# rishabhgoel0213/ZeroClone

Hardware: AMD Instinct MI355X
Metric: MCTS node-expansions/sec (whole node), Connect4 800 sims/move at 1/2/4/8 MI355X (higher is better)
Workload: dtype f64

## Files before the change

zeroclone_amd/csrc/c4_device.h:

```cpp
#pragma once
#include <math.h>

#include "c4_order_table.h"
#include "zc_internal.h"

namespace zc {
namespace {

__constant__ uint32_t d_order[128] = {ZC_C4_ORDER_LIST};

constexpr uint32_t kRingMask = kRingWords - 1;
constexpr uint64_t kBottom = 0x0000040810204081ull;
constexpr uint64_t kFull = kBottom * 0x3Full;
constexpr uint64_t kTop = kBottom << 5;
constexpr int kTabBytes = 128 * 4 + 128 * 8;

__device__ __forceinline__ uint32_t untried_init(uint32_t n) { return ((1u << n) - 1u) | (n << 28); }
__device__ __forceinline__ uint32_t untried_count(uint32_t u) { return (uint32_t)__popc(u & 0x7Fu); }

__device__ __forceinline__ void load_tables(uint32_t *s_order) {
    for (int i = (int)threadIdx.x; i < 128; i += blockDim.x) s_order[i] = d_order[i];
    uint8_t *const s_sel = (uint8_t *)(s_order + 128);
    for (int i = (int)threadIdx.x; i < 1024; i += blockDim.x) {
        const uint32_t m = (uint32_t)i >> 3, r = (uint32_t)i & 7u;
        uint32_t c = 0, pos = 7;
        for (uint32_t b = 0; b < 7; ++b)
            if ((m >> b) & 1u) {
                if (c == r) {
                    pos = b;
                    break;
                }
                ++c;
            }
        s_sel[i] = (uint8_t)pos;
    }
}
__device__ __forceinline__ const uint8_t *sel_table(const uint32_t *s_order) { return (const uint8_t *)(s_order + 128); }
constexpr int kWin = 64;
constexpr int kPathSpill = 2 * (64 - kMaxDepth) + 24;

__device__ __forceinline__ uint32_t uni(uint32_t x) { return (uint32_t)__builtin_amdgcn_readfirstlane((int)x); }
__device__ __forceinline__ int uni(int x) { return __builtin_amdgcn_readfirstlane(x); }
__device__ __forceinline__ uint64_t uni64(uint64_t x) {
    return ((uint64_t)uni((uint32_t)(x >> 32)) << 32) | (uint64_t)uni((uint32_t)x);
}
__device__ __forceinline__ uint32_t lane_id() { return __lane_id(); }
__device__ __forceinline__ uint32_t mask_sel(uint64_t m, uint32_t a, uint32_t b) {
    uint32_t r;
    __asm__("v_cndmask_b32 %0, %1, %2, %3" : "=v"(r) : "v"(a), "v"(b), "s"(m));
    return r;
}
__device__ __forceinline__ uint32_t mask_sel0(uint64_t m, uint32_t b) {
// ... 152 lines not shown

__device__ __forceinline__ uint32_t rng_view(const Rng &r) {
    const uint32_t lane = lane_id();
    const uint32_t src = lane < r.off ? r.wn : r.wt;
    return (uint32_t)__builtin_amdgcn_ds_bpermute((int)((lane + r.off) << 2), (int)src);
}

__device__ __forceinline__ void rng_close(const Rng &r, uint64_t use0, uint64_t *rngpos) {
    rngpos[0] = use0 + (uint64_t)(int64_t)r.use();
    rngpos[1] = use0 + (uint64_t)(int64_t)r.grel;
}

constexpr int kLRingWords = 1024;
constexpr uint32_t kLRingMask = kLRingWords - 1;
constexpr int kLRingBytes = kLRingWords * 4;

struct LRng {
    uint32_t *lds;
    uint32_t base;
    int32_t wrel;
    uint32_t off;
    int32_t hrel;
    uint32_t wa, wb;
    uint64_t ph;
    __device__ __forceinline__ uint32_t cur() const { return mask_sel(ph, wa, wb); }
    uint32_t wx;
    uint32_t ia, ib, im;
    __device__ __forceinline__ int32_t use() const { return wrel + (int32_t)off; }
    __device__ __forceinline__ uint32_t slot(int32_t rel) const { return (base + (uint32_t)rel) & kLRingMask; }
};

__device__ __forceinline__ uint32_t mt_twist(uint32_t a, uint32_t b, uint32_t m) {
    const uint32_t y = (a & 0x80000000u) | (b & 0x7fffffffu);
    return m ^ (y >> 1) ^ ((b & 1u) ? 0x9908b0dfu : 0u);
}

__device__ __forceinline__ void lrng_prefetch(LRng &r) {
    const int32_t p = r.wrel + 192 + (int32_t)lane_id();
    r.ia = r.lds[r.slot(p - 624)];
    r.ib = r.lds[r.slot(p - 623)];
    r.im = r.lds[r.slot(p - 227)];
}

__device__ __forceinline__ void lrng_generate_abs(uint32_t *lds, uint64_t g, uint64_t end) {
    const uint32_t lane = lane_id();
    for (; g < end; g += 64) {
        const uint32_t p = (uint32_t)g + lane;
        const uint32_t a = lds[(p - 624) & kLRingMask], b = lds[(p - 623) & kLRingMask],
                       m = lds[(p - 227) & kLRingMask];
        if (g + lane < end) lds[p & kLRingMask] = mt_twist(a, b, m);
        wave_mem_order();
    }
}

__device__ __forceinline__ void lrng_open(LRng &r, uint32_t *lds, const uint32_t *ring, uint64_t use0, uint64_t gen0) {
    const uint32_t lane = lane_id();
    r.lds = lds;
    r.base = (uint32_t)use0;
    r.off = (uint32_t)use0 & (uint32_t)(kWin - 1);
    r.wrel = -(int32_t)r.off;
    const uint64_t w0 = use0 - r.off, target = w0 + 192;
    const uint64_t g = gen0 <= w0 + 960 ? gen0 : (target < 624 ? 624 : target);
    for (uint32_t i = lane; i < (uint32_t)kLRingWords; i += 64) {
        const uint32_t p = (uint32_t)g - (uint32_t)kLRingWords + i;
        lds[p & kLRingMask] = ring[p & kRingMask];
    }
    wave_mem_order();
    lrng_generate_abs(lds, g, target);
    r.hrel = (int32_t)(g - use0);
    r.wa = temper(lds[r.slot(r.wrel + (int32_t)lane)]);
    r.wb = temper(lds[r.slot(r.wrel + kWin + (int32_t)lane)]);
    r.ph = 0;
    r.wx = lds[r.slot(r.wrel + 2 * kWin + (int32_t)lane)];
    lrng_prefetch(r);
}

__device__ __forceinline__ uint32_t rng_view(const LRng &r) {
    const uint32_t lane = lane_id();
    const uint32_t src = mask_sel(__ballot(lane < r.off) ^ r.ph, r.wa, r.wb);
    return (uint32_t)__builtin_amdgcn_ds_bpermute((int)((lane + r.off) << 2), (int)src);
}

__device__ __forceinline__ void rng_advance(LRng &r) {
    r.wrel += kWin;
    r.off -= (uint32_t)kWin;
    const uint32_t t = temper(r.wx);
    const uint32_t na = mask_sel(r.ph, t, r.wa), nb = mask_sel(r.ph, r.wb, t);
    r.wa = na;
    r.wb = nb;
    r.ph = ~r.ph;
    const int32_t p = r.wrel + 128 + (int32_t)lane_id();
    uint32_t x = mt_twist(r.ia, r.ib, r.im);
    if (r.wrel + 128 < r.hrel) {
        const uint32_t old = r.lds[r.slot(p)];
        x = p < r.hrel ? old : x;
    }
    r.lds[r.slot(p)] = x;
    r.wx = x;
    lrng_prefetch(r);
}

__device__ __forceinline__ void lrng_skip(LRng &r, uint32_t w) {
    r.off += w;
    while (r.off >= (uint32_t)kWin) rng_advance(r);
}

__device__ __forceinline__ void lrng_close(const LRng &r, uint32_t *ring, uint64_t use0, uint64_t *rngpos) {
    const uint32_t lane = lane_id();
    const uint64_t U = use0 + (uint64_t)(int64_t)r.use();
    uint64_t G = use0 + (uint64_t)(int64_t)max(r.wrel + 192, r.hrel);
    const uint64_t blk = U ? (U - 1) / 624 : 0;
    const uint64_t bend = (blk + 1) * 624;
    wave_mem_order();
    if (G < bend) {
        lrng_generate_abs(r.lds, G, bend);
        G = bend;
    }
    const uint64_t wu = U & ~(uint64_t)(kWin - 1);
    uint64_t start = wu < blk * 624 ? wu : blk * 624;
    start = start < G - 624 ? start : G - 624;
    for (uint64_t q = start + lane; q < G; q += 64) ring[(uint32_t)q & kRingMask] = r.lds[(uint32_t)q & kLRingMask];
    if (lane == 0) {
        rngpos[0] = U;
        rngpos[1] = G;
    }
}

template <class R>
__device__ __forceinline__ uint32_t rng_below(R &r, uint32_t n) {
    const uint32_t sh = (uint32_t)__clz(n);
    const uint32_t lane = lane_id();
    for (;;) {
        if (r.off >= (uint32_t)kWin) rng_advance(r);
        const uint32_t v = r.cur() >> sh;
        const uint64_t bal = __ballot((v | ((lane - r.off) & 0x80000000u)) < n);
        if (bal) {
// ... 254 lines not shown
            if (lane == (uint32_t)depth) pathv = (uint32_t)child | ((uint32_t)s << 16);
            node = child;
            ow = (uint32_t)__builtin_amdgcn_readlane((int)c_low, i);
            cmask = __builtin_amdgcn_readlane((int)c_lmask, i);
            u = untried_init((ow >> 24) & 15u);
            ul = kIdentList;
            ch = 0xFFFF;
            stamp.mark(2);
            continue;
        }
        const int m = min((int)cnt, nb - j);
        uint32_t rr = 0;
        {
            int done = 0;
            for (;;) {
                if (rng.off >= (uint32_t)kWin) rng_advance(rng);
                const uint32_t w = rng_view(rng);
                const int rem = m - done;
                uint64_t A[7];
#pragma unroll
                for (int i = 0; i < 7; ++i) {
                    const uint32_t n = (uint32_t)max((int)cnt - done - i, 1);
                    A[i] = __ballot((w >> __clz(n)) < n);
                }
                uint64_t gt = ~0ull, F = 0;
#pragma unroll
                for (int i = 0; i < 7; ++i) {
                    const uint64_t acc = (i < rem ? A[i] : 0ull) & gt;
                    const uint64_t lb = acc & (0ull - acc);
                    F |= lb;
                    gt = 0ull - (lb << 1);
                }
                const int nd = __popcll(F);
                const int f = 63 - __clzll(F | 1ull);
                const uint32_t di = (uint32_t)done + mbcnt64(F);
                const uint32_t rl = w >> __clz(max((int)cnt - (int)di, 1));
                const uint32_t got = (uint32_t)__builtin_amdgcn_ds_permute((int)(mask_sel(F, 63u, di) << 2), (int)rl);
                rr = mask_sel(((1ull << nd) - 1ull) << done, rr, got);
                done += nd;
                if (done < m) {
                    rng.off += (uint32_t)kWin;
                    continue;
                }
                rng.off += (uint32_t)f + 1u;
                break;
            }
        }
        uint32_t pl = rr;
        uint32_t rpick[6];
#pragma unroll
        for (int i = 0; i < 6; ++i) rpick[i] = (uint32_t)__builtin_amdgcn_readlane((int)rr, i);
#pragma unroll
        for (int i = 5; i >= 0; --i) {
            const uint64_t later = ((1ull << m) - 1ull) & ~((2ull << i) - 1ull);
            pl = add_in_mask(pl, __ballot(pl >= rpick[i]) & later);
        }
        const uint32_t mi_l = (ul >> (3 * (pl & 7u))) & 7u;
        uint32_t slotbit = (int)lane < m ? 1u << mi_l : 0u;
        slotbit |= (uint32_t)dpp<0xB1>((int)slotbit);
// ... 68 lines not shown
```

zeroclone_amd/csrc/c4_ext.hip:

```cpp
#include <hip/hip_fp16.h>

#include "c4_device.h"

namespace zc {
namespace {

__device__ __forceinline__ uint32_t mbcnt_lo(uint64_t m) {
    return __builtin_amdgcn_mbcnt_hi((uint32_t)(m >> 32), __builtin_amdgcn_mbcnt_lo((uint32_t)m, 0u));
}

__device__ __forceinline__ Tree ext_tree(const ExtParams &p, int g) {
    return Tree{p.a.nodes + (size_t)g * p.M * kRecBytes};
}

__global__ __launch_bounds__(kBlock) void c4_ext_begin_kernel(ExtParams p) {
    const uint32_t lane = lane_id();
    const int gl = blockIdx.x;
    if (gl >= p.n_games) return;
    const int g = p.first_game + gl;
    const zc_c4_state root = p.roots[gl];
    const uint64_t rp0 = uni64(root.stones[0]), rp1 = uni64(root.stones[1]);
    const int rturn = uni(root.turn);
    int status = 0;
    if (!valid_state(rp0, rp1, rturn)) status = ZC_STATUS_BAD_STATE;
// ... 332 lines not shown
}

void launch_c4_hp_walk(const ExtParams &p, hipStream_t s) {
    hipLaunchKernelGGL(c4_hp_walk_kernel, dim3(1), dim3(kBlock), 0, s, p);
}

void launch_c4_hp_expand(const ExtParams &p, hipStream_t s) {
    hipLaunchKernelGGL(c4_hp_expand_kernel, dim3(1), dim3(kBlock), 0, s, p);
}

void launch_c4_ext_begin(const ExtParams &p, hipStream_t s) {
    hipLaunchKernelGGL(c4_ext_begin_kernel, dim3(p.n_games), dim3(kBlock), 0, s, p);
}

void launch_c4_ext_select(const ExtParams &p, hipStream_t s) {
    hipLaunchKernelGGL(c4_ext_select_kernel, dim3(p.n_games), dim3(kBlock), c4_search_lds_bytes(p.bs), s, p);
}

void launch_c4_ext_backup(const ExtParams &p, hipStream_t s) {
    const size_t lds = (sizeof(double) + sizeof(int32_t)) * (size_t)p.bs;
    hipLaunchKernelGGL(c4_ext_backup_kernel, dim3(p.n_games), dim3(kBlock), lds, s, p);
}

void launch_c4_ext_end(const ExtParams &p, hipStream_t s) {
    hipLaunchKernelGGL(c4_ext_end_kernel, dim3(p.n_games), dim3(kBlock), 0, s, p);
}

}
```

zeroclone_amd/csrc/c4_search.hip:

```cpp
#include "c4_device.h"
#include "counter_rng.h"

namespace zc {
namespace {


__device__ __forceinline__ uint64_t readlane64(uint64_t x, int l) {
    return ((uint64_t)(uint32_t)__builtin_amdgcn_readlane((int)(x >> 32), l) << 32) |
           (uint64_t)(uint32_t)__builtin_amdgcn_readlane((int)x, l);
}

__device__ __forceinline__ uint32_t mbcnt(uint64_t m) {
    return __builtin_amdgcn_mbcnt_hi((uint32_t)(m >> 32), __builtin_amdgcn_mbcnt_lo((uint32_t)m, 0u));
}

__device__ __forceinline__ uint32_t scan_add32(uint32_t x) {
    x += (uint32_t)__builtin_amdgcn_update_dpp(0, (int)x, 0x111, 0xF, 0xF, false);
    x += (uint32_t)__builtin_amdgcn_update_dpp(0, (int)x, 0x112, 0xF, 0xF, false);
    x += (uint32_t)__builtin_amdgcn_update_dpp(0, (int)x, 0x114, 0xF, 0xF, false);
    x += (uint32_t)__builtin_amdgcn_update_dpp(0, (int)x, 0x118, 0xF, 0xF, false);
    x += (uint32_t)__builtin_amdgcn_update_dpp(0, (int)x, 0x142, 0xA, 0xF, false);
    x += (uint32_t)__builtin_amdgcn_update_dpp(0, (int)x, 0x143, 0xC, 0xF, false);
    return x;
}
// ... 44 lines not shown
    do {                                                            \
        if (ZC_RSTAMP && sub) {                                     \
            __builtin_amdgcn_sched_barrier(0);                      \
            const uint64_t now_ = __builtin_amdgcn_s_memtime();     \
            __builtin_amdgcn_sched_barrier(0);                      \
            if (ZC_RSTAMP == (k)) *sub += now_ - t_;                \
            t_ = now_;                                              \
        }                                                           \
    } while (0)
template <class R>
__device__ void c4_rollouts(Leaf *L, int nb, R &rng, const uint32_t *s_order, Counters &cn,
                            uint64_t *sub = nullptr) {
    uint64_t t_ = ZC_RSTAMP && sub ? __builtin_amdgcn_s_memtime() : 0;
    const uint32_t lane = lane_id();
    const uint32_t lrow = lane >> 4;
    const uint64_t second_rows = __ballot((lrow & 1u) != 0);
    const uint32_t d1 = lrow < 2 ? 1u : 6u, d2 = lrow < 2 ? 7u : 8u;
    const uint32_t pairbits = lane < 49u ? (1u << (lane / 7u)) | (1u << (lane % 7u)) : 0u;
    __builtin_amdgcn_s_waitcnt(0x0F70);
    for (int g = 0; g < nb; g += 64) {
      uint32_t lm_v = 0, ow_v = 0, hp_v = 0;
      int room_v = 0;
      int val_v = 0, q_v = 0;
      {
        const int jj = g + (int)lane;
        if (jj < nb) {
            lm_v = L[jj].meta;
            ow_v = L[jj].ow;
            const uint64_t x0 = L[jj].p0, x1 = L[jj].p1;
            const uint64_t op_v = (lm_v >> 24) & 1u ? x0 : x1;
            room_v = has_four(op_v) ? -2 : 41 - __popcll(x0 | x1);
            const uint64_t oc = x0 | x1;
            for (int c = 0; c < 7; ++c) hp_v |= (uint32_t)__popcll((oc >> (7 * c)) & 0x3Full) << (4 * c);
#ifndef ZC_DIAG_WASTE
            cn.blocks += room_v >= 0 ? 1 : 0;
#endif
        }
      }
      const int jend = min(nb, g + 64);
      for (int j = g; j < jend; ++j) {
        RMARK(6);
        const int jl = j - g;
        const uint32_t lm = (uint32_t)__builtin_amdgcn_readlane((int)lm_v, jl);
        uint4 pw;
        __builtin_memcpy(&pw, &L[j], sizeof pw);
        uint64_t x0 = ((uint64_t)pw.y << 32) | pw.x, x1 = ((uint64_t)pw.w << 32) | pw.z;
        uint64_t S1 = (lm >> 24) & 1u ? ~second_rows : second_rows;
        uint32_t hp = (uint32_t)__builtin_amdgcn_readlane((int)hp_v, jl);
        const uint32_t low0 = (uint32_t)__builtin_amdgcn_readlane((int)ow_v, jl);
        const int room0 = __builtin_amdgcn_readlane(room_v, jl);
        int val = (room0 + 1) >> 1;
        int q = 0;
        RMARK(1);
        if (room0 >= 0) {
            int room = room0;
            int mask = (int)(lm >> 25);
            uint32_t ow = low0;
            uint32_t n = (ow >> 24) & 15u;
            uint32_t sh = (uint32_t)__builtin_clz(n);
            uint32_t owp = s_order[(uint32_t)mask & ~pairbits];
            uint32_t ew, l0, lf, endlane, endply, col, sc;
            uint64_t F, mine;
            auto block = [&]() __attribute__((always_inline)) {
                RMARK(6);
                uint32_t wv, v;
                uint64_t A;
                if (rng.off >= (uint32_t)kWin) rng_advance(rng);
                wv = rng_view(rng);
                v = wv >> sh;
                A = __ballot(v < n);
                if (__builtin_expect(A == 0ull, 0)) {
                    do {
                        rng.off += (uint32_t)kWin;
                        rng_advance(rng);
                        wv = rng_view(rng);
                        v = wv >> sh;
                        A = __ballot(v < n);
                    } while (A == 0ull);
                }
                RMARK(2);
                const uint32_t cap_r = min((uint32_t)room, 30u);
                uint32_t qk = mbcnt(A);
                col = (ow >> (3 * v)) & 7u;
                uint32_t one = mask_sel0(A, 1u << (4 * col));
                sc = scan_add32(one);
                uint32_t row = ((sc - one + hp) >> (4 * col)) & 15u;
                uint32_t nacc = (uint32_t)__popcll(A);
                F = __ballot(row == 5u);
                uint64_t E0 = A & (F | __ballot(qk >= min(cap_r, nacc - 1u)));
                l0 = (uint32_t)__builtin_ctzll(E0);
                const uint64_t G = A & F & __ballot(qk < cap_r);
                lf = ff1(G);
#ifdef ZC_DIAG_WASTE
                const uint32_t l0f = l0;
#endif
#if !(ZC_RV & 1)
                RMARK(3);
                if (lf == l0) {
                    const uint32_t cf = (uint32_t)__builtin_amdgcn_readlane((int)col, (int)lf);
                    const uint32_t ow2 = (uint32_t)__builtin_amdgcn_readlane((int)owp, (int)(8u * cf));
                    const uint32_t n2 = (ow2 >> 24) & 15u;
                    const uint32_t v2 = wv >> __clz(n2);
                    const uint64_t high = ~1ull << lf;
                    A = (A & ~high) | (__ballot(v2 < n2) & high);
                    qk = mbcnt(A);
                    col = mask_sel(high, col, (ow2 >> (3 * v2)) & 7u);
                    one = mask_sel0(A, 1u << (4 * col));
                    sc = scan_add32(one);
                    row = ((sc - one + hp) >> (4 * col)) & 15u;
                    nacc = (uint32_t)__popcll(A);
                    F = __ballot(row == 5u) & high;
                    E0 = A & (F | __ballot(qk >= min(cap_r, nacc - 1u)));
                    l0 = (uint32_t)__builtin_ctzll(E0);
                }
                RMARK(4);
                const uint32_t c = ((qk & 1u) << 4) | ((qk >> 1) & 15u) | (qk & 32u);
                const uint32_t b = __umul24(col, 7u) + row;
                const uint32_t pl = (uint32_t)__builtin_amdgcn_ds_permute((int)(mask_sel(A, 63u, c) << 2), (int)b);
                const uint32_t pb = __builtin_amdgcn_permlane32_swap(pl, pl, false, false)[0];
                const uint64_t bit = 1ull << (pb & 63u);
                uint32_t blo = (uint32_t)bit, bhi = (uint32_t)(bit >> 32);
// ... 21 lines not shown
                    x0 = in_vgpr(x0);
                    x1 = in_vgpr(x1);
                    const uint64_t bd = (((uint64_t)mask_sel(S1, (uint32_t)(x0 >> 32), (uint32_t)(x1 >> 32)) << 32) |
                                         mask_sel(S1, (uint32_t)x0, (uint32_t)x1)) | mine_;
                    const uint64_t m1 = bd & (bd >> d1), m2 = bd & (bd >> d2);
                    const uint64_t f4 = (m1 & (m1 >> (2 * d1))) | (m2 & (m2 >> (2 * d2)));
                    const uint64_t W = __ballot(f4 != 0ull);
                    const uint32_t W32 = (uint32_t)W | (uint32_t)(W >> 32);
                    return A_ & __ballot(((W32 >> (c & 31u)) & 1u) != 0u);
                };
                uint64_t Ew1 = 0, mine1 = 0;
                RMARK(3);
                if (lf == l0) {
                    const uint32_t cf = (uint32_t)__builtin_amdgcn_readlane((int)col, (int)lf);
                    const uint32_t ow2 = (uint32_t)__builtin_amdgcn_readlane((int)owp, (int)(8u * cf));
                    const uint32_t n2 = (ow2 >> 24) & 15u;
                    const uint32_t v2 = wv >> __clz(n2);
                    const uint64_t high = ~1ull << lf;
                    if (ZC_RV & 1) Ew1 = win_test(A, qk, col, row, mine1) & ~high;
                    A = (A & ~high) | (__ballot(v2 < n2) & high);
                    qk = mbcnt(A);
                    col = mask_sel(high, col, (ow2 >> (3 * v2)) & 7u);
                    one = mask_sel0(A, 1u << (4 * col));
                    sc = scan_add32(one);
                    row = ((sc - one + hp) >> (4 * col)) & 15u;
                    nacc = (uint32_t)__popcll(A);
                    F = __ballot(row == 5u) & high;
                    E0 = A & (F | __ballot(qk >= min(cap_r, nacc - 1u)));
                    l0 = (uint32_t)__builtin_ctzll(E0);
                }
                RMARK(4);
                uint64_t Ew;
                if ((ZC_RV & 1) && Ew1 != 0ull) {
                    Ew = Ew1;
                    mine = mine1;
                } else {
                    Ew = win_test(A, qk, col, row, mine);
                }
                if (ZC_RV & 1) Ew = uni64(Ew);
#endif
                ew = ff1(Ew);
                endlane = min(ew, l0);
                endply = (uint32_t)__builtin_amdgcn_readlane((int)qk, (int)endlane);
                rng.off += endlane + 1u;
#ifdef ZC_DIAG_WASTE
                cn.add(cn.blocks, lf == l0f && endlane < lf ? 1 : 0);
                cn.add(cn.plies, lf == l0f ? 1 : 0);
#endif
                room -= (int)endply + 1;
                RMARK(5);
                return neg_if_le(ew, l0, room);
            };
            auto go_on = [&]() __attribute__((always_inline)) {
#ifndef ZC_DIAG_WASTE
                cn.add(cn.blocks, 1);
#endif
                {
                    const uint64_t s2 = readlane64(mine, (int)((endply + 31u) >> 1));
                    const uint64_t a2 = readlane64(mine, (int)(endply >> 1));
// ... 1 lines not shown
                    const bool p1_first = S1 & 1ull;
                    x0 |= p1_first ? b2 : a2;
                    x1 |= p1_first ? a2 : b2;
                    S1 = endply & 1u ? S1 : ~S1;
                }
                hp += (uint32_t)__builtin_amdgcn_readlane((int)sc, (int)endlane);
                const bool fa = endlane >= lf;
                const bool fe = (F >> endlane) & 1u;
                {
                    const uint32_t ca = (uint32_t)__builtin_amdgcn_readlane((int)col, (int)(fa ? lf : endlane));
                    const uint32_t ce = fe ? (uint32_t)__builtin_amdgcn_readlane((int)col, (int)endlane) : ca;
                    const bool ff = fa | fe;
                    mask = ff ? mask & ~((1 << ca) | (1 << ce)) : mask;
                    const uint32_t ownew = (uint32_t)__builtin_amdgcn_readlane((int)owp, (int)((7u * ca + ce) & 63u));
                    ow = ff ? ownew : ow;
                    owp = s_order[(uint32_t)mask & ~pairbits];
                }
                n = (ow >> 24) & 15u;
                sh = (uint32_t)__builtin_clz(n);
            };
            if (block() >= 0) {
                do go_on();
                while (block() >= 0);
            }
            q = room0 - room;
            val = ew <= l0 ? ((q & 1) ? 1 : -1) : 0;
        }
        val_v = zc_writelane(val, jl, val_v);
        q_v = zc_writelane(q, jl, q_v);
      }
      if (g + (int)lane < jend) L[g + (int)lane].val = val_v;
#ifndef ZC_DIAG_WASTE
      cn.plies += q_v;
#endif
// ... 167 lines not shown
        return;
    }

    constexpr uint32_t kIdentList = 0x1AC688u;
    uint64_t b0 = we.b0, b1 = we.b1;
    int turn = we.turn, depth = we.depth;
    uint32_t ow = we.ow, cm = (uint32_t)legal_mask(b0 | b1), n = cnt0, ul = 0;
    {
        uint32_t k = 0;
        for (uint32_t bb = 0; bb < 7; ++bb)
            if ((we.u >> bb) & 1u) ul |= bb << (3 * k++);
    }
    int d = 0, i = 0, T = -1;
    uint64_t Sm = 0;
    uint32_t raw = 0;
    if (rng.off >= (uint32_t)kWin) rng_advance(rng);
    uint32_t w = rng_view(rng);
    uint32_t t3 = w >> 29;
    uint64_t gt = ~0ull, Fv = 0;
    int dv0 = 0;
    for (;;) {
        const int m = min((int)n, nb - d);
        if (lane == 0)
            chain[i] = ChainNode{b0, b1, ow,
                                 n | ((uint32_t)m << 4) | ((uint32_t)d << 8) | ((uint32_t)depth << 16) |
                                     ((uint32_t)turn << 24) | (cm << 25),
                                 ul, 0u};
        if (m == 0) {
            T = i;
            break;
        }
        Sm |= 1ull << d;
        int k = 0;
// ... 7 lines not shown
#pragma unroll
            for (int s = 0; s < 7; ++s) {
                const uint64_t acc = A[s] & gt;
                gt = (~1ull) << (ff1(acc) & 63u);
                F |= acc & ~gt;
            }
            Fv |= F;
            const int nd = __popcll(F);
            k += nd;
            d += nd;
            if (k < m) {
                const uint32_t di = (uint32_t)dv0 + mbcnt64(Fv);
                const uint32_t got =
                    (uint32_t)__builtin_amdgcn_ds_permute((int)(mask_sel(Fv, 63u, di) << 2), (int)w);
                raw = mask_sel(lanes_in(dv0, d), raw, got);
                rng.off += (uint32_t)kWin;
                rng_advance(rng);
                w = rng_view(rng);
                t3 = w >> 29;
                gt = ~0ull;
                Fv = 0;
                dv0 = d;
                continue;
            }
            gt = (~1ull) << (63 - __clzll(Fv));
            break;
        }
        if (d >= nb) break;
        const int col = (int)((ow >> (3 * (ul & 7u))) & 7u);
        const uint64_t bit = drop_bit(b0 | b1, col);
        if (turn) b1 |= bit; else b0 |= bit;
        turn ^= 1;
        ++depth;
        if (bit & kTop) {
            cm &= ~(1u << col);
            ow = uni(s_order[cm]);
        }
        n = (ow >> 24) & 15u;
        ul = kIdentList;
        ++i;
    }
    {
        const uint32_t di = (uint32_t)dv0 + mbcnt64(Fv);
        const uint32_t got = (uint32_t)__builtin_amdgcn_ds_permute((int)(mask_sel(Fv, 63u, di) << 2), (int)w);
        raw = mask_sel(lanes_in(dv0, d), raw, got);
        rng.off += (uint32_t)(63 - __clzll(Fv | 1ull)) + 1u;
    }
    const int D = d;
    wave_mem_order();
    stamp.mark(2);

    const bool act = (int)lane < D;
    const uint32_t seg = act ? mbcnt64(Sm) + (uint32_t)((Sm >> lane) & 1ull) - 1u : 0u;
    const ChainNode e = chain[seg];
    const uint32_t s_i = (e.info >> 8) & 0xFFu;
    const uint32_t dd = lane - s_i;
    const uint32_t r = raw >> __clz(act ? (e.info & 15u) - dd : 1u);
    uint32_t rp[6];
#pragma unroll
    for (int s = 0; s < 6; ++s) rp[s] = (uint32_t)__builtin_amdgcn_ds_bpermute((int)((s_i + (uint32_t)s) << 2), (int)r);
    uint32_t pl = r;
#pragma unroll
    for (int s = 5; s >= 0; --s) pl += (dd > (uint32_t)s && pl >= rp[s]) ? 1u : 0u;
    const uint32_t mi = (e.ul >> (3 * (pl & 7u))) & 7u;
    const uint64_t Z = __ballot(act && pl == 0);
    const uint64_t zl = Z & ((1ull << s_i) - 1ull);
    const int parent = seg == 0 ? we.node : f0 + 63 - __clzll(zl | 1ull);
    {
        const uint32_t col = (e.ow >> (3 * mi)) & 7u;
        const uint64_t bit = drop_bit(e.p0 | e.p1, (int)col);
        const uint32_t tn = (e.info >> 24) & 1u, ldepth = ((e.info >> 16) & 0xFFu) + 1u;
        const bool filled = (bit & kTop) != 0;
// ... 38 lines not shown
            const int q = base + (int)lane;
            const uint32_t dep = q < D ? fresh[q].link >> 24 : 0u;
#pragma unroll
            for (int bit = 0; bit < 6; ++bit) dsum += __popcll(__ballot((dep >> bit) & 1u)) << bit;
        }
        cn.add(cn.expansions, D);
        cn.add(cn.depth_sum, dsum);
    }
    stamp.mark(3);
}

__device__ __forceinline__ uint32_t draw_class_bfe(uint32_t cnt) {
    return (6u << 16) | (((0xE480u >> (2u * cnt)) & 3u) << 3);
}

__device__ __forceinline__ uint32_t draw_table(uint32_t w) {
    const uint32_t lane = lane_id();
    const uint32_t t3 = lane < 62u ? (w >> 29) : 7u;
    uint32_t nx = 0;
#pragma unroll
    for (uint32_t c = 0; c < 4; ++c) {
        const uint64_t s = __ballot(t3 < 4u + c) >> lane;
        const uint32_t f = s ? lane + 1u + (uint32_t)__builtin_ctzll(s) : 63u;
        nx |= f << (8u * c);
    }
    return nx;
}

__device__ __forceinline__ void write_lane(int &v, uint32_t x, int i) {
    __asm__("v_writelane_b32 %0, %1, m0" : "+v"(v) : "s"(x), "{m0}"(i));
}

__device__ __forceinline__ uint32_t draw_step(uint32_t nx, uint32_t q, uint32_t op) {
// ... 87 lines not shown
        ++i;
    }
    const int D = d;

    const bool act = (int)lane < D;
    const uint32_t seg = act ? mbcnt64(Sm) + (uint32_t)((Sm >> lane) & 1ull) - 1u : 0u;
    const int sa = (int)(seg << 2);
    const uint32_t e_cd = (uint32_t)__builtin_amdgcn_ds_bpermute(sa, v_cd);
    const uint32_t s_i = (e_cd >> 8) & 0xFFu;
    const uint32_t dd = lane - s_i;
    const uint32_t cnt = act ? (e_cd >> 16) - dd : 1u;
    const uint32_t clsv = draw_class_bfe(act ? cnt : 1u);

    uint32_t raw = 0;
    {
        if (rng.off >= (uint32_t)kWin) rng_advance(rng);
        uint32_t w = rng_view(rng);
        uint32_t nx = draw_table(w);
        int V = 0;
        uint64_t F = draw_chase_fixed<32>(nx, clsv);
        for (;;) {
            const uint64_t Fv = F & 0x7FFFFFFFFFFFFFFEull;
            const uint64_t G = Fv >> 1;
            const int nv = __popcll(G), need = D - V, take = min(nv, need);
            const uint32_t rank = mbcnt64(G);
            const bool send = ((G >> lane) & 1ull) && (int)rank < take;
            const uint32_t got = (uint32_t)__builtin_amdgcn_ds_permute(
                (int)((send ? (uint32_t)V + rank : 63u) << 2), (int)w);
            raw = mask_sel(lanes_in(V, V + take), raw, got);
            V += take;
            if (nv >= need) {
                const uint64_t lastw = __ballot(((G >> lane) & 1ull) && (int)rank == take - 1);
                rng.off += (uint32_t)__builtin_ctzll(lastw) + 1u;
                break;
            }
            uint32_t q;
            if (F >> 63) {
                rng.off += 62u;
                if (rng.off >= (uint32_t)kWin) rng_advance(rng);
                w = rng_view(rng);
                nx = draw_table(w);
                q = 0;
            } else {
                q = nv ? 64u - (uint32_t)__clzll(G) : 0u;
                rng.off += q;
                if (rng.off >= (uint32_t)kWin) rng_advance(rng);
                w = rng_view(rng);
                nx = draw_table(w);
                q = 0;
            }
            F = 0;
            for (int k = V; k < D; ++k) {
                q = draw_step(nx, q, (uint32_t)__builtin_amdgcn_readlane((int)clsv, k));
                F |= 1ull << q;
                if (q == 63u) break;
            }
        }
    }
    wave_mem_order();
    stamp.mark(2);

    const uint32_t e_ow = (uint32_t)__builtin_amdgcn_ds_bpermute(sa, v_ow);
    const uint64_t e_p0 = ((uint64_t)(uint32_t)__builtin_amdgcn_ds_bpermute(sa, v_b0h) << 32) |
                          (uint32_t)__builtin_amdgcn_ds_bpermute(sa, v_b0l);
    const uint64_t e_p1 = ((uint64_t)(uint32_t)__builtin_amdgcn_ds_bpermute(sa, v_b1h) << 32) |
                          (uint32_t)__builtin_amdgcn_ds_bpermute(sa, v_b1l);
    const uint32_t r = raw >> __clz(cnt);
    uint32_t rp[6];
#pragma unroll
    for (int s = 0; s < 6; ++s) rp[s] = (uint32_t)__builtin_amdgcn_ds_bpermute((int)((s_i + (uint32_t)s) << 2), (int)r);
    uint32_t pl = r;
#pragma unroll
    for (int s = 5; s >= 0; --s) pl += (dd > (uint32_t)s && pl >= rp[s]) ? 1u : 0u;
    const uint32_t mi = seg == 0 ? (uint32_t)sel_table(s_order)[8u * (we.u & 0x7Fu) + (pl & 7u)] : pl;
    const uint64_t Z = __ballot(act && pl == 0);
    const uint64_t zl = Z & ((1ull << s_i) - 1ull);
    const int parent = seg == 0 ? we.node : f0 + 63 - __clzll(zl | 1ull);
    {
        const uint32_t col = (e_ow >> (3 * mi)) & 7u;
        const uint64_t bit = drop_bit(e_p0 | e_p1, (int)col);
        const uint32_t tn = (uint32_t)we.turn ^ (seg & 1u), ldepth = (uint32_t)we.depth + seg + 1u;
        const bool filled = (bit & kTop) != 0;
// ... 42 lines not shown
    nnodes = f0 + D;
    wave_mem_order();
    {
        const uint32_t dep = act ? (uint32_t)we.depth + seg + 1u : 0u;
        int dsum = 0;
#pragma unroll
        for (int bit = 0; bit < 6; ++bit) dsum += __popcll(__ballot((dep >> bit) & 1u)) << bit;
        cn.add(cn.expansions, D);
        cn.add(cn.depth_sum, dsum);
    }
    stamp.mark(3);
}

constexpr int kSearchWaves = 4;
__host__ __device__ constexpr size_t c4_search_wave_lds(int bs) {
    return ((size_t)kLRingBytes + (sizeof(Leaf) + sizeof(Fresh) + sizeof(uint16_t) * kMaxDepth) * (size_t)bs +
            kPathSpill + 15) & ~(size_t)15;
}

struct SearchLds {
    uint32_t *s_order;
    uint32_t *ring;
    Fresh *fresh;
    Leaf *leaves;
    uint16_t *paths;
};

__device__ __forceinline__ SearchLds search_lds(uint8_t *s_dyn, int bs) {
    const uint32_t wave = threadIdx.x >> 6;
    uint8_t *const s_wave = s_dyn + kTabBytes + (size_t)wave * c4_search_wave_lds(bs);
    SearchLds L;
    L.s_order = (uint32_t *)s_dyn;
    L.ring = (uint32_t *)s_wave;
    L.fresh = (Fresh *)(s_wave + kLRingBytes);
    L.leaves = (Leaf *)(s_wave + kLRingBytes + sizeof(Fresh) * (size_t)bs);
    L.paths = (uint16_t *)(s_wave + kLRingBytes + (sizeof(Fresh) + sizeof(Leaf)) * (size_t)bs);
    return L;
}

template <bool STAMP, bool PHILOX, int WALK = 0>
__device__ __forceinline__ void search_move(const SearchParams &p, const SearchLds &L, int gl, int g, const Tree &t,
                                            LRng &rng, uint32_t tag, Counters &cn, int &status, int &done_io,
                                            int &nnodes_io, const int32_t *stop = nullptr, int32_t budget = 0,
                                            int *lagp = nullptr, const int32_t *progress = nullptr, int mv = 0) {
    int lag = lagp ? *lagp : 0;
    const uint32_t lane = lane_id();
    const uint32_t *const s_order = L.s_order;
    Fresh *const fresh = L.fresh;
    Leaf *const leaves = L.leaves;
    ConstDouble *logtab = (ConstDouble *)p.a.logtab;
    if (done_io == 0) {
// ... 11 lines not shown

        FlushSel fs;
        {
            const zc_c4_state root = p.roots[gl];
#ifndef ZC_NO_PLAN
#define ZC_NO_PLAN 0
#endif
#ifndef ZC_PLAN2
#define ZC_PLAN2 1
#endif
            if (!ZC_NO_PLAN && ZC_PLAN2 && p.bs < 64)
                select_flush_plan2<STAMP>(t, fresh, leaves, s_order, logtab, rng, cn, stamp, nnodes, status,
                                          uni64(root.stones[0]), uni64(root.stones[1]), uni(root.turn), done, nb,
                                          p.c, fs);
            else if (!ZC_NO_PLAN && p.bs < 64)
                select_flush_plan<STAMP>(t, fresh, leaves, (ChainNode *)L.paths, s_order, logtab, rng, cn, stamp,
                                         nnodes, status, uni64(root.stones[0]), uni64(root.stones[1]),
                                         uni(root.turn), done, nb, p.c, fs);
            else
                select_flush<false, STAMP>(t, fresh, leaves, nullptr, s_order, logtab, rng, cn, stamp, nnodes,
                                           status, uni64(root.stones[0]), uni64(root.stones[1]), uni(root.turn),
                                           done, nb, p.c, fs);
        }
        const int f0 = fs.f0, d0 = fs.d0;

        const size_t wlog = (size_t)g * p.sims + done;
        const size_t wfl = (size_t)g * ((p.sims + p.bs - 1) / p.bs) + done / p.bs;
        if (WALK == 2) {
            for (int jj = (int)lane; jj < nb; jj += kBlock) leaves[jj].val = p.walk_vals[wlog + jj];
            lrng_skip(rng, uni(p.walk_words[wfl]));
        } else if (PHILOX) {
// ... 540 lines not shown
```

Baseline: 3.436 billion.

## Precompute 3-bit tempered draws in LDS and refill MT ring in 4-word steps

Replaces the register-windowed Mersenne Twister reader with an LDS byte array of pre-tempered 3-bit draws (top bits of temper), so consumers read one byte per lane instead of tempering and bpermuting full words. The ring is refilled in batched steps of 224 words with 4 words per lane, and a new draw-order table is built at load time so move selection compares 3-bit draws against thresholds directly. It also changes the per-wave LDS layout and sizing. The cost is extra LDS per wave and more work in each refill step, which may limit occupancy; the ext_select launch now computes its LDS size separately from the shared helper.

```diff
diff --git a/zeroclone_amd/csrc/c4_device.h b/zeroclone_amd/csrc/c4_device.h
--- a/zeroclone_amd/csrc/c4_device.h
+++ b/zeroclone_amd/csrc/c4_device.h
@@ -13,13 +13,20 @@
 constexpr uint64_t kBottom = 0x0000040810204081ull;
 constexpr uint64_t kFull = kBottom * 0x3Full;
 constexpr uint64_t kTop = kBottom << 5;
-constexpr int kTabBytes = 128 * 4 + 128 * 8;
+constexpr int kTabBytes = 128 * 4 + 128 * 8 + 128 * 4;
 
 __device__ __forceinline__ uint32_t untried_init(uint32_t n) { return ((1u << n) - 1u) | (n << 28); }
 __device__ __forceinline__ uint32_t untried_count(uint32_t u) { return (uint32_t)__popc(u & 0x7Fu); }
 
 __device__ __forceinline__ void load_tables(uint32_t *s_order) {
-    for (int i = (int)threadIdx.x; i < 128; i += blockDim.x) s_order[i] = d_order[i];
+    for (int i = (int)threadIdx.x; i < 128; i += blockDim.x) {
+        const uint32_t o = d_order[i], n = (o >> 24) & 15u;
+        s_order[i] = o;
+        const uint32_t sh = n ? (uint32_t)__builtin_clz(n) - 29u : 0u;
+        uint32_t e = (n << sh) << 24;
+        for (uint32_t t = 0; t < (n << sh); ++t) e |= ((o >> (3u * (t >> sh))) & 7u) << (3u * t);
+        s_order[128 + 256 + i] = e;
+    }
     uint8_t *const s_sel = (uint8_t *)(s_order + 128);
     for (int i = (int)threadIdx.x; i < 1024; i += blockDim.x) {
         const uint32_t m = (uint32_t)i >> 3, r = (uint32_t)i & 7u;
@@ -36,6 +43,7 @@
     }
 }
 __device__ __forceinline__ const uint8_t *sel_table(const uint32_t *s_order) { return (const uint8_t *)(s_order + 128); }
+__device__ __forceinline__ const uint32_t *draw_order_table(const uint32_t *s_order) { return s_order + 128 + 256; }
 constexpr int kWin = 64;
 constexpr int kPathSpill = 2 * (64 - kMaxDepth) + 24;
 
@@ -218,35 +226,78 @@
 constexpr int kLRingWords = 1024;
 constexpr uint32_t kLRingMask = kLRingWords - 1;
 constexpr int kLRingBytes = kLRingWords * 4;
+constexpr int kLDrawBytes = kLRingWords + kWin;
+constexpr int kLStepLanes = 56;
+constexpr int kLStep = 4 * kLStepLanes;
+static_assert(kLStep <= 227 && kLStep % 4 == 0, "a refill step's inputs must all be older than its outputs");
+static_assert(kLRingWords - 624 - (kWin - 1 + kLStep) >= 0, "the block of word U-1 must stay in the ring");
+
+__host__ __device__ constexpr uint32_t mt_draw3(uint32_t x) {
+    const uint32_t y = x ^ (x >> 11);
+    const uint32_t z = y ^ ((y << 7) & 0x80004000u);
+    return (z ^ (z << 15)) >> 29;
+}
+__host__ __device__ constexpr uint32_t mt_temper_ref(uint32_t y) {
+    y ^= y >> 11;
+    y ^= (y << 7) & 0x9d2c5680u;
+    y ^= (y << 15) & 0xefc60000u;
+    y ^= y >> 18;
+    return y;
+}
+__host__ __device__ constexpr bool mt_draw3_matches_temper() {
+    if (mt_draw3(0u) != mt_temper_ref(0u) >> 29) return false;
+    for (int b = 0; b < 32; ++b)
+        if (mt_draw3(1u << b) != mt_temper_ref(1u << b) >> 29) return false;
+    return true;
+}
+static_assert(mt_draw3_matches_temper(), "mt_draw3 is not temper(x) >> 29");
 
 struct LRng {
     uint32_t *lds;
-    uint32_t base;
-    int32_t wrel;
-    uint32_t off;
-    int32_t hrel;
-    uint32_t wa, wb;
-    uint64_t ph;
-    __device__ __forceinline__ uint32_t cur() const { return mask_sel(ph, wa, wb); }
-    uint32_t wx;
-    uint32_t ia, ib, im;
-    __device__ __forceinline__ int32_t use() const { return wrel + (int32_t)off; }
-    __device__ __forceinline__ uint32_t slot(int32_t rel) const { return (base + (uint32_t)rel) & kLRingMask; }
+    const uint8_t *dl;
+    int32_t urel;
+    int32_t lim;
+    int32_t uoff;
+    __device__ __forceinline__ int32_t use() const { return urel - uoff; }
+    __device__ __forceinline__ int32_t grel() const { return lim + kWin; }
+    __device__ __forceinline__ uint8_t *draw() const { return (uint8_t *)(lds + kLRingWords); }
 };
 
 __device__ __forceinline__ uint32_t mt_twist(uint32_t a, uint32_t b, uint32_t m) {
-    const uint32_t y = (a & 0x80000000u) | (b & 0x7fffffffu);
-    return m ^ (y >> 1) ^ ((b & 1u) ? 0x9908b0dfu : 0u);
-}
-
-__device__ __forceinline__ void lrng_prefetch(LRng &r) {
-    const int32_t p = r.wrel + 192 + (int32_t)lane_id();
-    r.ia = r.lds[r.slot(p - 624)];
-    r.ib = r.lds[r.slot(p - 623)];
-    r.im = r.lds[r.slot(p - 227)];
-}
-
-__device__ __forceinline__ void lrng_generate_abs(uint32_t *lds, uint64_t g, uint64_t end) {
+    uint32_t y;
+    __asm__("v_bfi_b32 %0, %1, %2, %3" : "=v"(y) : "s"(0x7fffffffu), "v"(b), "v"(a));
+    const uint32_t mag = (uint32_t)((int32_t)(b << 31) >> 31) & 0x9908b0dfu;
+    return m ^ (y >> 1) ^ mag;
+}
+
+__device__ __forceinline__ void lrng_put_draws(const LRng &r, uint32_t q, uint32_t x0, uint32_t x1, uint32_t x2,
+                                               uint32_t x3) {
+    const uint32_t d = mt_draw3(x0) | (mt_draw3(x1) << 8) | (mt_draw3(x2) << 16) | (mt_draw3(x3) << 24);
+    *(uint32_t *)(r.draw() + q) = d;
+    if (q < (uint32_t)kWin) *(uint32_t *)(r.draw() + kLRingWords + q) = d;
+}
+
+__device__ __forceinline__ void lrng_refill(LRng &r) {
+    const uint32_t lane = lane_id();
+    const uint32_t p = (uint32_t)r.grel() + 4u * lane;
+    const uint32_t *pa = r.lds + ((p - 624u) & kLRingMask), *pm = r.lds + ((p - 228u) & kLRingMask);
+    const uint32_t a0 = pa[0], a1 = pa[1], a2 = pa[2], a3 = pa[3], a4 = r.lds[(p - 620u) & kLRingMask];
+    const uint32_t m1 = pm[1], m2 = pm[2], m3 = pm[3], m4 = r.lds[(p - 224u) & kLRingMask];
+    const uint32_t x0 = mt_twist(a0, a1, m1), x1 = mt_twist(a1, a2, m2), x2 = mt_twist(a2, a3, m3),
+                   x3 = mt_twist(a3, a4, m4);
+    if (lane < (uint32_t)kLStepLanes) {
+        uint32_t *px = r.lds + (p & kLRingMask);
+        px[0] = x0;
+        px[1] = x1;
+        px[2] = x2;
+        px[3] = x3;
+        lrng_put_draws(r, p & kLRingMask, x0, x1, x2, x3);
+    }
+    r.lim += kLStep;
+    wave_mem_order();
+}
+
+__device__ __forceinline__ void lrng_generate(uint32_t *lds, int64_t g, int64_t end) {
     const uint32_t lane = lane_id();
     for (; g < end; g += 64) {
         const uint32_t p = (uint32_t)g + lane;
@@ -259,71 +310,74 @@
 
 __device__ __forceinline__ void lrng_open(LRng &r, uint32_t *lds, const uint32_t *ring, uint64_t use0, uint64_t gen0) {
     const uint32_t lane = lane_id();
+    const uint64_t org = use0 & ~(uint64_t)3;
     r.lds = lds;
-    r.base = (uint32_t)use0;
-    r.off = (uint32_t)use0 & (uint32_t)(kWin - 1);
-    r.wrel = -(int32_t)r.off;
-    const uint64_t w0 = use0 - r.off, target = w0 + 192;
-    const uint64_t g = gen0 <= w0 + 960 ? gen0 : (target < 624 ? 624 : target);
+    r.dl = r.draw() + lane;
+    r.uoff = (int32_t)(use0 - org);
+    r.urel = r.uoff;
+    const uint64_t w0 = use0 & ~(uint64_t)(kWin - 1), target = w0 + 192;
+    uint64_t g = gen0 <= w0 + 960 ? gen0 : (target < 624 ? 624 : target);
     for (uint32_t i = lane; i < (uint32_t)kLRingWords; i += 64) {
         const uint32_t p = (uint32_t)g - (uint32_t)kLRingWords + i;
-        lds[p & kLRingMask] = ring[p & kRingMask];
+        lds[(p - (uint32_t)org) & kLRingMask] = ring[p & kRingMask];
     }
     wave_mem_order();
-    lrng_generate_abs(lds, g, target);
-    r.hrel = (int32_t)(g - use0);
-    r.wa = temper(lds[r.slot(r.wrel + (int32_t)lane)]);
-    r.wb = temper(lds[r.slot(r.wrel + kWin + (int32_t)lane)]);
-    r.ph = 0;
-    r.wx = lds[r.slot(r.wrel + 2 * kWin + (int32_t)lane)];
-    lrng_prefetch(r);
-}
-
-__device__ __forceinline__ uint32_t rng_view(const LRng &r) {
-    const uint32_t lane = lane_id();
-    const uint32_t src = mask_sel(__ballot(lane < r.off) ^ r.ph, r.wa, r.wb);
-    return (uint32_t)__builtin_amdgcn_ds_bpermute((int)((lane + r.off) << 2), (int)src);
-}
-
-__device__ __forceinline__ void rng_advance(LRng &r) {
-    r.wrel += kWin;
-    r.off -= (uint32_t)kWin;
-    const uint32_t t = temper(r.wx);
-    const uint32_t na = mask_sel(r.ph, t, r.wa), nb = mask_sel(r.ph, r.wb, t);
-    r.wa = na;
-    r.wb = nb;
-    r.ph = ~r.ph;
-    const int32_t p = r.wrel + 128 + (int32_t)lane_id();
-    uint32_t x = mt_twist(r.ia, r.ib, r.im);
-    if (r.wrel + 128 < r.hrel) {
-        const uint32_t old = r.lds[r.slot(p)];
-        x = p < r.hrel ? old : x;
-    }
-    r.lds[r.slot(p)] = x;
-    r.wx = x;
-    lrng_prefetch(r);
-}
+    if (g < use0 + kWin || (g & 3u)) {
+        const uint64_t ge = ((g < use0 + kWin ? use0 + kWin : g) + 3u) & ~(uint64_t)3u;
+        lrng_generate(lds, (int64_t)(g - org), (int64_t)(ge - org));
+        g = ge;
+    }
+    for (uint32_t q = 4u * lane; q < (uint32_t)kLRingWords; q += 256u)
+        lrng_put_draws(r, q, lds[q], lds[q + 1], lds[q + 2], lds[q + 3]);
+    wave_mem_order();
+    r.lim = (int32_t)(int64_t)(g - org) - kWin;
+}
+
+__device__ __forceinline__ uint32_t rng_view(const LRng &r) { return r.dl[(uint32_t)r.urel & kLRingMask]; }
 
 __device__ __forceinline__ void lrng_skip(LRng &r, uint32_t w) {
-    r.off += w;
-    while (r.off >= (uint32_t)kWin) rng_advance(r);
+    r.urel += (int32_t)w;
+    while (r.urel > r.lim) lrng_refill(r);
+}
+
+__device__ __forceinline__ void rng_need(Rng &r) {
+    if (r.off >= (uint32_t)kWin) rng_advance(r);
+}
+__device__ __forceinline__ void rng_need(LRng &r) {
+    if (r.urel > r.lim) lrng_refill(r);
+}
+__device__ __forceinline__ void rng_eat(Rng &r, uint32_t w) { r.off += w; }
+__device__ __forceinline__ void rng_eat(LRng &r, uint32_t w) { r.urel += (int32_t)w; }
+template <class R>
+struct ViewBits {
+    static constexpr uint32_t kBits = 32;
+};
+template <>
+struct ViewBits<LRng> {
+    static constexpr uint32_t kBits = 3;
+};
+template <class R>
+__device__ __forceinline__ uint32_t draw_shift(uint32_t n) {
+    return (uint32_t)__builtin_clz(n) - (32u - ViewBits<R>::kBits);
 }
 
 __device__ __forceinline__ void lrng_close(const LRng &r, uint32_t *ring, uint64_t use0, uint64_t *rngpos) {
     const uint32_t lane = lane_id();
-    const uint64_t U = use0 + (uint64_t)(int64_t)r.use();
-    uint64_t G = use0 + (uint64_t)(int64_t)max(r.wrel + 192, r.hrel);
+    const uint64_t org = use0 & ~(uint64_t)3;
+    const uint64_t U = org + (uint64_t)(int64_t)r.urel;
+    uint64_t G = org + (uint64_t)(int64_t)r.grel();
     const uint64_t blk = U ? (U - 1) / 624 : 0;
     const uint64_t bend = (blk + 1) * 624;
     wave_mem_order();
     if (G < bend) {
-        lrng_generate_abs(r.lds, G, bend);
+        lrng_generate(r.lds, (int64_t)(G - org), (int64_t)(bend - org));
         G = bend;
     }
     const uint64_t wu = U & ~(uint64_t)(kWin - 1);
     uint64_t start = wu < blk * 624 ? wu : blk * 624;
     start = start < G - 624 ? start : G - 624;
-    for (uint64_t q = start + lane; q < G; q += 64) ring[(uint32_t)q & kRingMask] = r.lds[(uint32_t)q & kLRingMask];
+    for (uint64_t q = start + lane; q < G; q += 64)
+        ring[(uint32_t)q & kRingMask] = r.lds[((uint32_t)q - (uint32_t)org) & kLRingMask];
     if (lane == 0) {
         rngpos[0] = U;
         rngpos[1] = G;
@@ -608,14 +662,14 @@
         {
             int done = 0;
             for (;;) {
-                if (rng.off >= (uint32_t)kWin) rng_advance(rng);
+                rng_need(rng);
                 const uint32_t w = rng_view(rng);
                 const int rem = m - done;
                 uint64_t A[7];
 #pragma unroll
                 for (int i = 0; i < 7; ++i) {
                     const uint32_t n = (uint32_t)max((int)cnt - done - i, 1);
-                    A[i] = __ballot((w >> __clz(n)) < n);
+                    A[i] = __ballot((w >> draw_shift<RNG>(n)) < n);
                 }
                 uint64_t gt = ~0ull, F = 0;
 #pragma unroll
@@ -628,15 +682,15 @@
                 const int nd = __popcll(F);
                 const int f = 63 - __clzll(F | 1ull);
                 const uint32_t di = (uint32_t)done + mbcnt64(F);
-                const uint32_t rl = w >> __clz(max((int)cnt - (int)di, 1));
+                const uint32_t rl = w >> draw_shift<RNG>((uint32_t)max((int)cnt - (int)di, 1));
                 const uint32_t got = (uint32_t)__builtin_amdgcn_ds_permute((int)(mask_sel(F, 63u, di) << 2), (int)rl);
                 rr = mask_sel(((1ull << nd) - 1ull) << done, rr, got);
                 done += nd;
                 if (done < m) {
-                    rng.off += (uint32_t)kWin;
+                    rng_eat(rng, (uint32_t)kWin);
                     continue;
                 }
-                rng.off += (uint32_t)f + 1u;
+                rng_eat(rng, (uint32_t)f + 1u);
                 break;
             }
         }
diff --git a/zeroclone_amd/csrc/c4_ext.hip b/zeroclone_amd/csrc/c4_ext.hip
--- a/zeroclone_amd/csrc/c4_ext.hip
+++ b/zeroclone_amd/csrc/c4_ext.hip
@@ -370,7 +370,8 @@
 }
 
 void launch_c4_ext_select(const ExtParams &p, hipStream_t s) {
-    hipLaunchKernelGGL(c4_ext_select_kernel, dim3(p.n_games), dim3(kBlock), c4_search_lds_bytes(p.bs), s, p);
+    const size_t lds = kTabBytes + (sizeof(Fresh) + sizeof(Leaf) + sizeof(uint16_t) * kMaxDepth) * (size_t)p.bs + kPathSpill;
+    hipLaunchKernelGGL(c4_ext_select_kernel, dim3(p.n_games), dim3(kBlock), lds, s, p);
 }
 
 void launch_c4_ext_backup(const ExtParams &p, hipStream_t s) {
diff --git a/zeroclone_amd/csrc/c4_search.hip b/zeroclone_amd/csrc/c4_search.hip
--- a/zeroclone_amd/csrc/c4_search.hip
+++ b/zeroclone_amd/csrc/c4_search.hip
@@ -82,6 +82,8 @@
     uint64_t t_ = ZC_RSTAMP && sub ? __builtin_amdgcn_s_memtime() : 0;
     const uint32_t lane = lane_id();
     const uint32_t lrow = lane >> 4;
+    constexpr uint32_t kTop3 = ViewBits<R>::kBits - 3u;
+    const uint32_t *const s_dorder = draw_order_table(s_order);
     const uint64_t second_rows = __ballot((lrow & 1u) != 0);
     const uint32_t d1 = lrow < 2 ? 1u : 6u, d2 = lrow < 2 ? 7u : 8u;
     const uint32_t pairbits = lane < 49u ? (1u << (lane / 7u)) | (1u << (lane % 7u)) : 0u;
@@ -94,7 +96,7 @@
         const int jj = g + (int)lane;
         if (jj < nb) {
             lm_v = L[jj].meta;
-            ow_v = L[jj].ow;
+            ow_v = s_dorder[lm_v >> 25];
             const uint64_t x0 = L[jj].p0, x1 = L[jj].p1;
             const uint64_t op_v = (lm_v >> 24) & 1u ? x0 : x1;
             room_v = has_four(op_v) ? -2 : 41 - __popcll(x0 | x1);
@@ -124,32 +126,29 @@
             int room = room0;
             int mask = (int)(lm >> 25);
             uint32_t ow = low0;
-            uint32_t n = (ow >> 24) & 15u;
-            uint32_t sh = (uint32_t)__builtin_clz(n);
-            uint32_t owp = s_order[(uint32_t)mask & ~pairbits];
+            uint32_t thr = (ow >> 24) & 15u;
+            uint32_t owp = s_dorder[(uint32_t)mask & ~pairbits];
             uint32_t ew, l0, lf, endlane, endply, col, sc;
             uint64_t F, mine;
             auto block = [&]() __attribute__((always_inline)) {
                 RMARK(6);
-                uint32_t wv, v;
+                uint32_t wv;
                 uint64_t A;
-                if (rng.off >= (uint32_t)kWin) rng_advance(rng);
-                wv = rng_view(rng);
-                v = wv >> sh;
-                A = __ballot(v < n);
+                rng_need(rng);
+                wv = rng_view(rng) >> kTop3;
+                A = __ballot(wv < thr);
                 if (__builtin_expect(A == 0ull, 0)) {
                     do {
-                        rng.off += (uint32_t)kWin;
-                        rng_advance(rng);
-                        wv = rng_view(rng);
-                        v = wv >> sh;
-                        A = __ballot(v < n);
+                        rng_eat(rng, (uint32_t)kWin);
+                        rng_need(rng);
+                        wv = rng_view(rng) >> kTop3;
+                        A = __ballot(wv < thr);
                     } while (A == 0ull);
                 }
                 RMARK(2);
                 const uint32_t cap_r = min((uint32_t)room, 30u);
                 uint32_t qk = mbcnt(A);
-                col = (ow >> (3 * v)) & 7u;
+                col = (ow >> (3 * wv)) & 7u;
                 uint32_t one = mask_sel0(A, 1u << (4 * col));
                 sc = scan_add32(one);
                 uint32_t row = ((sc - one + hp) >> (4 * col)) & 15u;
@@ -167,12 +166,11 @@
                 if (lf == l0) {
                     const uint32_t cf = (uint32_t)__builtin_amdgcn_readlane((int)col, (int)lf);
                     const uint32_t ow2 = (uint32_t)__builtin_amdgcn_readlane((int)owp, (int)(8u * cf));
-                    const uint32_t n2 = (ow2 >> 24) & 15u;
-                    const uint32_t v2 = wv >> __clz(n2);
+                    const uint32_t thr2 = (ow2 >> 24) & 15u;
                     const uint64_t high = ~1ull << lf;
-                    A = (A & ~high) | (__ballot(v2 < n2) & high);
+                    A = (A & ~high) | (__ballot(wv < thr2) & high);
                     qk = mbcnt(A);
-                    col = mask_sel(high, col, (ow2 >> (3 * v2)) & 7u);
+                    col = mask_sel(high, col, (ow2 >> (3 * wv)) & 7u);
                     one = mask_sel0(A, 1u << (4 * col));
                     sc = scan_add32(one);
                     row = ((sc - one + hp) >> (4 * col)) & 15u;
@@ -224,13 +222,12 @@
                 if (lf == l0) {
                     const uint32_t cf = (uint32_t)__builtin_amdgcn_readlane((int)col, (int)lf);
                     const uint32_t ow2 = (uint32_t)__builtin_amdgcn_readlane((int)owp, (int)(8u * cf));
-                    const uint32_t n2 = (ow2 >> 24) & 15u;
-                    const uint32_t v2 = wv >> __clz(n2);
+                    const uint32_t thr2 = (ow2 >> 24) & 15u;
                     const uint64_t high = ~1ull << lf;
                     if (ZC_RV & 1) Ew1 = win_test(A, qk, col, row, mine1) & ~high;
-                    A = (A & ~high) | (__ballot(v2 < n2) & high);
+                    A = (A & ~high) | (__ballot(wv < thr2) & high);
                     qk = mbcnt(A);
-                    col = mask_sel(high, col, (ow2 >> (3 * v2)) & 7u);
+                    col = mask_sel(high, col, (ow2 >> (3 * wv)) & 7u);
                     one = mask_sel0(A, 1u << (4 * col));
                     sc = scan_add32(one);
                     row = ((sc - one + hp) >> (4 * col)) & 15u;
@@ -252,7 +249,7 @@
                 ew = ff1(Ew);
                 endlane = min(ew, l0);
                 endply = (uint32_t)__builtin_amdgcn_readlane((int)qk, (int)endlane);
-                rng.off += endlane + 1u;
+                rng_eat(rng, endlane + 1u);
 #ifdef ZC_DIAG_WASTE
                 cn.add(cn.blocks, lf == l0f && endlane < lf ? 1 : 0);
                 cn.add(cn.plies, lf == l0f ? 1 : 0);
@@ -284,10 +281,9 @@
                     mask = ff ? mask & ~((1 << ca) | (1 << ce)) : mask;
                     const uint32_t ownew = (uint32_t)__builtin_amdgcn_readlane((int)owp, (int)((7u * ca + ce) & 63u));
                     ow = ff ? ownew : ow;
-                    owp = s_order[(uint32_t)mask & ~pairbits];
+                    owp = s_dorder[(uint32_t)mask & ~pairbits];
                 }
-                n = (ow >> 24) & 15u;
-                sh = (uint32_t)__builtin_clz(n);
+                thr = (ow >> 24) & 15u;
             };
             if (block() >= 0) {
                 do go_on();
@@ -485,9 +481,9 @@
     int d = 0, i = 0, T = -1;
     uint64_t Sm = 0;
     uint32_t raw = 0;
-    if (rng.off >= (uint32_t)kWin) rng_advance(rng);
+    rng_need(rng);
     uint32_t w = rng_view(rng);
-    uint32_t t3 = w >> 29;
+    uint32_t t3 = w >> (ViewBits<RNG>::kBits - 3u);
     uint64_t gt = ~0ull, Fv = 0;
     int dv0 = 0;
     for (;;) {
@@ -525,10 +521,10 @@
                 const uint32_t got =
                     (uint32_t)__builtin_amdgcn_ds_permute((int)(mask_sel(Fv, 63u, di) << 2), (int)w);
                 raw = mask_sel(lanes_in(dv0, d), raw, got);
-                rng.off += (uint32_t)kWin;
-                rng_advance(rng);
+                rng_eat(rng, (uint32_t)kWin);
+                rng_need(rng);
                 w = rng_view(rng);
-                t3 = w >> 29;
+                t3 = w >> (ViewBits<RNG>::kBits - 3u);
                 gt = ~0ull;
                 Fv = 0;
                 dv0 = d;
@@ -555,7 +551,7 @@
         const uint32_t di = (uint32_t)dv0 + mbcnt64(Fv);
         const uint32_t got = (uint32_t)__builtin_amdgcn_ds_permute((int)(mask_sel(Fv, 63u, di) << 2), (int)w);
         raw = mask_sel(lanes_in(dv0, d), raw, got);
-        rng.off += (uint32_t)(63 - __clzll(Fv | 1ull)) + 1u;
+        rng_eat(rng, (uint32_t)(63 - __clzll(Fv | 1ull)) + 1u);
     }
     const int D = d;
     wave_mem_order();
@@ -566,7 +562,7 @@
     const ChainNode e = chain[seg];
     const uint32_t s_i = (e.info >> 8) & 0xFFu;
     const uint32_t dd = lane - s_i;
-    const uint32_t r = raw >> __clz(act ? (e.info & 15u) - dd : 1u);
+    const uint32_t r = raw >> draw_shift<RNG>(act ? (e.info & 15u) - dd : 1u);
     uint32_t rp[6];
 #pragma unroll
     for (int s = 0; s < 6; ++s) rp[s] = (uint32_t)__builtin_amdgcn_ds_bpermute((int)((s_i + (uint32_t)s) << 2), (int)r);
@@ -635,9 +631,9 @@
     return (6u << 16) | (((0xE480u >> (2u * cnt)) & 3u) << 3);
 }
 
-__device__ __forceinline__ uint32_t draw_table(uint32_t w) {
+__device__ __forceinline__ uint32_t draw_table(uint32_t w3) {
     const uint32_t lane = lane_id();
-    const uint32_t t3 = lane < 62u ? (w >> 29) : 7u;
+    const uint32_t t3 = lane < 62u ? w3 : 7u;
     uint32_t nx = 0;
 #pragma unroll
     for (uint32_t c = 0; c < 4; ++c) {
@@ -755,9 +751,9 @@
 
     uint32_t raw = 0;
     {
-        if (rng.off >= (uint32_t)kWin) rng_advance(rng);
+        rng_need(rng);
         uint32_t w = rng_view(rng);
-        uint32_t nx = draw_table(w);
+        uint32_t nx = draw_table(w >> (ViewBits<RNG>::kBits - 3u));
         int V = 0;
         uint64_t F = draw_chase_fixed<32>(nx, clsv);
         for (;;) {
@@ -772,22 +768,22 @@
             V += take;
             if (nv >= need) {
                 const uint64_t lastw = __ballot(((G >> lane) & 1ull) && (int)rank == take - 1);
-                rng.off += (uint32_t)__builtin_ctzll(lastw) + 1u;
+                rng_eat(rng, (uint32_t)__builtin_ctzll(lastw) + 1u);
                 break;
             }
             uint32_t q;
             if (F >> 63) {
-                rng.off += 62u;
-                if (rng.off >= (uint32_t)kWin) rng_advance(rng);
+                rng_eat(rng, 62u);
+                rng_need(rng);
                 w = rng_view(rng);
-                nx = draw_table(w);
+                nx = draw_table(w >> (ViewBits<RNG>::kBits - 3u));
                 q = 0;
             } else {
                 q = nv ? 64u - (uint32_t)__clzll(G) : 0u;
-                rng.off += q;
-                if (rng.off >= (uint32_t)kWin) rng_advance(rng);
+                rng_eat(rng, q);
+                rng_need(rng);
                 w = rng_view(rng);
-                nx = draw_table(w);
+                nx = draw_table(w >> (ViewBits<RNG>::kBits - 3u));
                 q = 0;
             }
             F = 0;
@@ -806,7 +802,7 @@
                           (uint32_t)__builtin_amdgcn_ds_bpermute(sa, v_b0l);
     const uint64_t e_p1 = ((uint64_t)(uint32_t)__builtin_amdgcn_ds_bpermute(sa, v_b1h) << 32) |
                           (uint32_t)__builtin_amdgcn_ds_bpermute(sa, v_b1l);
-    const uint32_t r = raw >> __clz(cnt);
+    const uint32_t r = raw >> draw_shift<RNG>(cnt);
     uint32_t rp[6];
 #pragma unroll
     for (int s = 0; s < 6; ++s) rp[s] = (uint32_t)__builtin_amdgcn_ds_bpermute((int)((s_i + (uint32_t)s) << 2), (int)r);
@@ -879,16 +875,18 @@
 
 constexpr int kSearchWaves = 4;
 __host__ __device__ constexpr size_t c4_search_wave_lds(int bs) {
-    return ((size_t)kLRingBytes + (sizeof(Leaf) + sizeof(Fresh) + sizeof(uint16_t) * kMaxDepth) * (size_t)bs +
-            kPathSpill + 15) & ~(size_t)15;
-}
+    return ((size_t)kLRingBytes + (size_t)kLDrawBytes + (sizeof(Leaf) + sizeof(Fresh)) * (size_t)bs +
+            sizeof(ChainNode) * ((size_t)bs + 1) + 15) & ~(size_t)15;
+}
+static_assert(c4_search_wave_lds(32) == 8800 && c4_search_wave_lds(32) <= 9536, "per-wave LDS at batch 32");
+static_assert(4 * (kTabBytes + kSearchWaves * c4_search_wave_lds(32)) <= 160 * 1024, "four workgroups per CU");
 
 struct SearchLds {
     uint32_t *s_order;
     uint32_t *ring;
     Fresh *fresh;
     Leaf *leaves;
-    uint16_t *paths;
+    ChainNode *chain;
 };
 
 __device__ __forceinline__ SearchLds search_lds(uint8_t *s_dyn, int bs) {
@@ -897,9 +895,10 @@
     SearchLds L;
     L.s_order = (uint32_t *)s_dyn;
     L.ring = (uint32_t *)s_wave;
-    L.fresh = (Fresh *)(s_wave + kLRingBytes);
-    L.leaves = (Leaf *)(s_wave + kLRingBytes + sizeof(Fresh) * (size_t)bs);
-    L.paths = (uint16_t *)(s_wave + kLRingBytes + (sizeof(Fresh) + sizeof(Leaf)) * (size_t)bs);
+    constexpr size_t kRings = (size_t)kLRingBytes + (size_t)kLDrawBytes;
+    L.fresh = (Fresh *)(s_wave + kRings);
+    L.leaves = (Leaf *)(s_wave + kRings + sizeof(Fresh) * (size_t)bs);
+    L.chain = (ChainNode *)(s_wave + kRings + (sizeof(Fresh) + sizeof(Leaf)) * (size_t)bs);
     return L;
 }
 
@@ -941,7 +940,7 @@
                                           uni64(root.stones[0]), uni64(root.stones[1]), uni(root.turn), done, nb,
                                           p.c, fs);
             else if (!ZC_NO_PLAN && p.bs < 64)
-                select_flush_plan<STAMP>(t, fresh, leaves, (ChainNode *)L.paths, s_order, logtab, rng, cn, stamp,
+                select_flush_plan<STAMP>(t, fresh, leaves, L.chain, s_order, logtab, rng, cn, stamp,
                                          nnodes, status, uni64(root.stones[0]), uni64(root.stones[1]),
                                          uni(root.turn), done, nb, p.c, fs);
             else
```

Result: faster. 3.610 billion, median of 6 (+5.1%).
